# ChenyangQiQi/FateZero

Hardware: NVIDIA H100
Metric: edited frames/sec (512x512x8f, 50 DDIM steps: inversion + attention-fused edit) (higher is better)
Workload: dtype f16 (fp32 accumulate)

## Files before the change

### fatezero_b200/_build.py

```python
from __future__ import annotations

import os
import subprocess
import sys

HERE = os.path.dirname(os.path.abspath(__file__))
CSRC = os.path.join(HERE, "csrc")
LIB = os.path.join(HERE, "libfatezero_b200.so")
SOURCES = ["fz_capi.cu", "fz_gemm.cu", "fz_elem.cu", "fz_attn.cu", "fz_p2p.cu", "fz_clip.cu"]
ARCH = ["-gencode", "arch=compute_90a,code=sm_90a"]
NVCC_FLAGS = [*ARCH, "-lineinfo", "-O3", "-std=c++17", "-Xcompiler", "-fPIC",
              "--use_fast_math" if False else "-DFZ_NO_FAST_MATH"]


def _nvcc() -> str:
    for cand in (os.environ.get("NVCC"), "/usr/local/cuda/bin/nvcc", "nvcc"):
        if cand and (os.path.isabs(cand) and os.path.exists(cand) or not os.path.isabs(cand)):
            return cand
    return "nvcc"


def needs_build() -> bool:
    if not os.path.exists(LIB):
        return True
    t = os.path.getmtime(LIB)
    deps = [os.path.join(CSRC, f) for f in os.listdir(CSRC)] + [os.path.join(HERE, "..", "include", "fatezero_b200.h")]
    return any(os.path.getmtime(d) > t for d in deps if os.path.exists(d))


def build(force: bool = False, verbose: bool = True, variant: str = "", extra_flags=()) -> str:
    if variant:
        return _build(os.path.join(HERE, f"libfatezero_b200_{variant}.so"), os.path.join(HERE, "build", variant), list(extra_flags), verbose)
    if not force and not needs_build():
        return LIB
    return _build(LIB, os.path.join(HERE, "build"), [], verbose)


def _build(lib: str, objdir: str, extra_flags, verbose: bool) -> str:
    objs = []
    procs = []
    os.makedirs(objdir, exist_ok=True)
    for src in SOURCES:
        obj = os.path.join(objdir, src.replace(".cu", ".o"))
        cmd = [_nvcc(), *NVCC_FLAGS, *extra_flags, "-c", os.path.join(CSRC, src), "-o", obj]
        if verbose:
            print(" ".join(cmd), flush=True)
        procs.append((src, subprocess.Popen(cmd, stdout=subprocess.PIPE, stderr=subprocess.STDOUT)))
        objs.append(obj)
    for src, p in procs:
        out, _ = p.communicate()
        if p.returncode != 0:
            raise RuntimeError(f"nvcc failed on {src}:\n{out.decode()}")
    cmd = [_nvcc(), "-shared", "-o", lib, *objs, *ARCH]
    if verbose:
        print(" ".join(cmd), flush=True)
    subprocess.check_call(cmd)
    return lib


if __name__ == "__main__":
    import argparse
    ap = argparse.ArgumentParser()
    ap.add_argument("--force", action="store_true")
    ap.add_argument("--variant", default="")
    ap.add_argument("--flags", default="")
    a = ap.parse_args()
    print(build(force=a.force, variant=a.variant, extra_flags=a.flags.split()))
```

### fatezero_b200/csrc/fz_common.cuh

```cuda
#pragma once
#include <cuda.h>
#include <cuda_fp16.h>
#include <cuda_runtime.h>
#include <stdint.h>
#include <stdio.h>

namespace fz {

void set_error(const char* fmt, ...);
int check_single_device();
#define FZ_OK 0
#define FZ_ERR_INVALID 1
#define FZ_ERR_CUDA 2
#define FZ_CHECK_ARG(cond, ...)                        \
  do {                                                 \
    if (!(cond)) {                                     \
      ::fz::set_error(__VA_ARGS__);                    \
      return FZ_ERR_INVALID;                           \
    }                                                  \
  } while (0)
#define FZ_CUDA(expr)                                                                           \
  do {                                                                                          \
    cudaError_t _e = (expr);                                                                    \
    if (_e != cudaSuccess) {                                                                    \
      ::fz::set_error("%s failed: %s (%s:%d)", #expr, cudaGetErrorString(_e), __FILE__, __LINE__); \
      return FZ_ERR_CUDA;                                                                       \
    }                                                                                           \
  } while (0)

#ifdef __CUDACC__

__device__ __forceinline__ uint32_t smem_u32(const void* p) { return static_cast<uint32_t>(__cvta_generic_to_shared(p)); }

__device__ __forceinline__ void pdl_wait() { asm volatile("griddepcontrol.wait;" ::: "memory"); }
__device__ __forceinline__ void pdl_launch_dependents() { asm volatile("griddepcontrol.launch_dependents;" ::: "memory"); }

__device__ __forceinline__ bool elect_one() {
  uint32_t pred = 0;
  asm volatile(
      "{\n\t.reg .pred P1;\n\telect.sync _|P1, 0xffffffff;\n\tselp.u32 %0, 1, 0, P1;\n\t}\n"
      : "=r"(pred));
  return pred != 0;
}

__device__ __forceinline__ void mbar_init(uint64_t* bar, uint32_t count) {
  asm volatile("mbarrier.init.shared::cta.b64 [%0], %1;" ::"r"(smem_u32(bar)), "r"(count) : "memory");
}
__device__ __forceinline__ void fence_mbar_init() { asm volatile("fence.mbarrier_init.release.cluster;" ::: "memory"); }
__device__ __forceinline__ void mbar_expect_tx(uint64_t* bar, uint32_t bytes) {
  asm volatile("mbarrier.arrive.expect_tx.shared::cta.b64 _, [%0], %1;" ::"r"(smem_u32(bar)), "r"(bytes) : "memory");
}
__device__ __forceinline__ void mbar_arrive(uint64_t* bar) {
  asm volatile("mbarrier.arrive.shared::cta.b64 _, [%0];" ::"r"(smem_u32(bar)) : "memory");
}
__device__ __forceinline__ bool mbar_try_wait(uint64_t* bar, uint32_t parity) {
  uint32_t ok;
  asm volatile(
      "{\n\t.reg .pred p;\n\tmbarrier.try_wait.parity.shared::cta.b64 p, [%1], %2;\n\tselp.u32 %0, 1, 0, p;\n\t}\n"
      : "=r"(ok)
      : "r"(smem_u32(bar)), "r"(parity)
      : "memory");
  return ok != 0;
}
#ifndef FZ_MBAR_TIMEOUT_NS
#define FZ_MBAR_TIMEOUT_NS 2000000000ull
#endif
__device__ __forceinline__ uint64_t global_timer_ns() {
  uint64_t t;
  asm volatile("mov.u64 %0, %%globaltimer;" : "=l"(t));
  return t;
}
__device__ __forceinline__ void mbar_wait(uint64_t* bar, uint32_t parity) {
  if (mbar_try_wait(bar, parity)) return;
  const uint64_t t0 = global_timer_ns();
  while (!mbar_try_wait(bar, parity))
    if (global_timer_ns() - t0 > FZ_MBAR_TIMEOUT_NS) __trap();
}

__device__ __forceinline__ void fence_proxy_async_smem() { asm volatile("fence.proxy.async.shared::cta;" ::: "memory"); }

__device__ __forceinline__ void tma_prefetch_desc(const CUtensorMap* m) {
  asm volatile("prefetch.tensormap [%0];" ::"l"(reinterpret_cast<uint64_t>(m)) : "memory");
}
__device__ __forceinline__ void tma_load_2d(void* dst, const CUtensorMap* m, uint64_t* bar, int c0, int c1) {
  asm volatile(
      "cp.async.bulk.tensor.2d.shared::cluster.global.mbarrier::complete_tx::bytes [%0], [%1, {%3, %4}], [%2];" ::"r"(
          smem_u32(dst)),
      "l"(reinterpret_cast<uint64_t>(m)), "r"(smem_u32(bar)), "r"(c0), "r"(c1)
      : "memory");
}
__device__ __forceinline__ void tma_load_3d(void* dst, const CUtensorMap* m, uint64_t* bar, int c0, int c1, int c2) {
  asm volatile(
      "cp.async.bulk.tensor.3d.shared::cluster.global.mbarrier::complete_tx::bytes [%0], [%1, {%3, %4, %5}], [%2];" ::"r"(
          smem_u32(dst)),
      "l"(reinterpret_cast<uint64_t>(m)), "r"(smem_u32(bar)), "r"(c0), "r"(c1), "r"(c2)
      : "memory");
}
__device__ __forceinline__ void tma_load_4d(void* dst, const CUtensorMap* m, uint64_t* bar, int c0, int c1, int c2, int c3) {
  asm volatile(
      "cp.async.bulk.tensor.4d.shared::cluster.global.mbarrier::complete_tx::bytes [%0], [%1, {%3, %4, %5, %6}], [%2];" ::"r"(
          smem_u32(dst)),
      "l"(reinterpret_cast<uint64_t>(m)), "r"(smem_u32(bar)), "r"(c0), "r"(c1), "r"(c2), "r"(c3)
      : "memory");
}
__device__ __forceinline__ void tma_load_5d(void* dst, const CUtensorMap* m, uint64_t* bar, int c0, int c1, int c2, int c3,
                                            int c4) {
  asm volatile(
      "cp.async.bulk.tensor.5d.shared::cluster.global.mbarrier::complete_tx::bytes [%0], [%1, {%3, %4, %5, %6, %7}], "
      "[%2];" ::"r"(smem_u32(dst)),
      "l"(reinterpret_cast<uint64_t>(m)), "r"(smem_u32(bar)), "r"(c0), "r"(c1), "r"(c2), "r"(c3), "r"(c4)
      : "memory");
}
__device__ __forceinline__ void tma_store_2d(const CUtensorMap* m, const void* src, int c0, int c1) {
  asm volatile("cp.async.bulk.tensor.2d.global.shared::cta.bulk_group [%0, {%2, %3}], [%1];" ::"l"(reinterpret_cast<uint64_t>(m)),
               "r"(smem_u32(src)), "r"(c0), "r"(c1)
               : "memory");
}
__device__ __forceinline__ void tma_store_4d(const CUtensorMap* m, const void* src, int c0, int c1, int c2, int c3) {
  asm volatile("cp.async.bulk.tensor.4d.global.shared::cta.bulk_group [%0, {%2, %3, %4, %5}], [%1];" ::"l"(
                   reinterpret_cast<uint64_t>(m)),
               "r"(smem_u32(src)), "r"(c0), "r"(c1), "r"(c2), "r"(c3)
               : "memory");
}
__device__ __forceinline__ void tma_store_5d(const CUtensorMap* m, const void* src, int c0, int c1, int c2, int c3, int c4) {
  asm volatile("cp.async.bulk.tensor.5d.global.shared::cta.bulk_group [%0, {%2, %3, %4, %5, %6}], [%1];" ::"l"(
                   reinterpret_cast<uint64_t>(m)),
               "r"(smem_u32(src)), "r"(c0), "r"(c1), "r"(c2), "r"(c3), "r"(c4)
               : "memory");
}
__device__ __forceinline__ void tma_store_commit() { asm volatile("cp.async.bulk.commit_group;" ::: "memory"); }
template <int N>
__device__ __forceinline__ void tma_store_wait_read() {
  asm volatile("cp.async.bulk.wait_group.read %0;" ::"n"(N) : "memory");
}
template <int N>
__device__ __forceinline__ void tma_store_wait_all() {
  asm volatile("cp.async.bulk.wait_group %0;" ::"n"(N) : "memory");
}

__device__ __forceinline__ uint64_t wgmma_desc_k_sw128(uint32_t smem_addr) {
  uint64_t d = 0;
  d |= static_cast<uint64_t>((smem_addr & 0x3FFFF) >> 4);
  d |= static_cast<uint64_t>(1) << 16;
  d |= static_cast<uint64_t>(1024 >> 4) << 32;
  d |= static_cast<uint64_t>(1) << 62;
  return d;
}
__device__ __forceinline__ void named_bar_sync(int id, int n) { asm volatile("bar.sync %0, %1;" ::"r"(id), "r"(n) : "memory"); }

#endif

template <typename... KArgs, typename... Args>
inline cudaError_t launch_pdl(void (*kernel)(KArgs...), dim3 grid, dim3 block, size_t smem, cudaStream_t stream, Args&&... args) {
  cudaLaunchConfig_t cfg = {};
  cfg.gridDim = grid;
  cfg.blockDim = block;
  cfg.dynamicSmemBytes = smem;
  cfg.stream = stream;
  cudaLaunchAttribute attr[1];
  attr[0].id = cudaLaunchAttributeProgrammaticStreamSerialization;
  attr[0].val.programmaticStreamSerializationAllowed = 1;
  cfg.attrs = attr;
  cfg.numAttrs = 1;
  return cudaLaunchKernelEx(&cfg, kernel, static_cast<KArgs>(args)...);
}

int encode_tmap_f16(CUtensorMap* out, const void* base, int rank, const uint64_t* dims, const uint64_t* strides_elems,
                    const uint32_t* box, bool swizzle128);
int encode_tmap_f16_sw(CUtensorMap* out, const void* base, int rank, const uint64_t* dims, const uint64_t* strides_elems,
                       const uint32_t* box, int swizzle_bytes);

}
```

### fatezero_b200/csrc/fz_gemm.cu

```cuda
#include "fz_common.cuh"
#include "fz_wgmma.cuh"

#include <algorithm>
#include <climits>
#include <cstdio>
#include <cstring>

#include "../../include/fatezero_b200.h"

namespace fz {

constexpr int kMaxTaps = 9;
constexpr int kBlockM = 128;
constexpr int kBlockK = 64;
constexpr int kATileBytes = kBlockM * kBlockK * 2;

struct TapGemmParams {
  CUtensorMap tmA;
  CUtensorMap tmB;
  CUtensorMap tmR[2];
  CUtensorMap tmE;
  int n_res;
  int res_kblocks;
  int a_rank;
  int M, N;
  int rows_per_tile;
  int a_box_bytes;
  int k_blocks;
  int num_taps;
  int n_tiles, m_tiles;
  int ndecomp;
  int dimsz[4];
  int tap_off[kMaxTaps][5];
  const float* bias;
  const float* group_bias;
  int rows_per_group;
  const __half* residual;
  long long ldr;
  const __half* residual2;
  long long ldr2;
  __half* out;
  long long ldo;
  int mode;
  int vt_col_start;
  __half* out_vt;
  int vt_S, vt_d, vt_heads, vt_ld;
};

template <int BLOCK_N>
struct TapGemmCfg {
  static constexpr int kBTileBytes = BLOCK_N * kBlockK * 2;
  static constexpr int kBTilePad = (kBTileBytes + 1023) / 1024 * 1024;
  static constexpr int kStageBytes = kATileBytes + kBTilePad;
  static constexpr int kStagesRaw = (227 * 1024 - 1280) / kStageBytes;
  static constexpr int kStages = kStagesRaw > 8 ? 8 : kStagesRaw;
  static constexpr int kSmemBytes = kStages * kStageBytes + 1024  + 256 ;
};

__device__ __forceinline__ float gelu_erf(float x) {
  const float z = fabsf(x) * 0.70710678118654752f;
  float t, e;
  asm("rcp.approx.ftz.f32 %0, %1;" : "=f"(t) : "f"(fmaf(0.3275911f, z, 1.0f)));
  float poly = fmaf(1.061405429f, t, -1.453152027f);
  poly = fmaf(poly, t, 1.421413741f);
  poly = fmaf(poly, t, -0.284496736f);
  poly = fmaf(poly, t, 0.254829592f);
  asm("ex2.approx.ftz.f32 %0, %1;" : "=f"(e) : "f"(-1.4426950408889634f * z * z));
  const float erf_abs = fmaf(-poly * t, e, 1.0f);
  return 0.5f * x * (1.0f + copysignf(erf_abs, x));
}

__device__ __forceinline__ void epi_store1(const TapGemmParams& p, long long m, int col, float v, const float* gb) {
  if (p.bias) v += __ldg(p.bias + col);
  if (col >= p.vt_col_start) {
    const long long bf = m / p.vt_S;
    const int s = static_cast<int>(m % p.vt_S);
    const int cv = col - p.vt_col_start;
    p.out_vt[((bf * p.vt_heads + cv / p.vt_d) * p.vt_d + cv % p.vt_d) * p.vt_ld + s] = __float2half_rn(v);
  } else {
    if (gb) v += __ldg(gb + col);
    if (p.residual) v += __half2float(p.residual[m * p.ldr + col]);
    if (p.residual2) v += __half2float(p.residual2[m * p.ldr2 + col]);
    p.out[m * p.ldo + col] = __float2half_rn(v);
  }
}

template <int BLOCK_N>
__global__ void __launch_bounds__(384, 1) tapgemm_kernel(const __grid_constant__ TapGemmParams p) {
  using Cfg = TapGemmCfg<BLOCK_N>;
  extern __shared__ uint8_t smem_raw[];
  uint8_t* smem = reinterpret_cast<uint8_t*>((reinterpret_cast<uintptr_t>(smem_raw) + 1023) & ~uintptr_t(1023));
  uint64_t* bars = reinterpret_cast<uint64_t*>(smem + Cfg::kStages * Cfg::kStageBytes);
  uint64_t* full = bars;
  uint64_t* empty = bars + Cfg::kStages;

  const int wg = threadIdx.x >> 7;
  pdl_launch_dependents();
  const int num_tiles = p.m_tiles * p.n_tiles;
  const int k_iters = p.num_taps * p.k_blocks + p.n_res * p.res_kblocks;

  if (threadIdx.x == 0) {
    tma_prefetch_desc(&p.tmA);
    tma_prefetch_desc(&p.tmB);
    for (int s = 0; s < Cfg::kStages; ++s) {
      mbar_init(&full[s], 1);
      mbar_init(&empty[s], 8);
    }
    fence_mbar_init();
  }
  __syncthreads();
  pdl_wait();

  if (wg == 2) {
    if (threadIdx.x == 256) {
      int stage = 0;
      uint32_t phase = 0;
      for (int tile = blockIdx.x; tile < num_tiles; tile += gridDim.x) {
        const int mt = tile / p.n_tiles, nt = tile % p.n_tiles;
        int rem = mt * p.rows_per_tile;
        int base[5] = {0, 0, 0, 0, 0};
        for (int d = 0; d < p.ndecomp; ++d) {
          base[d + 1] = rem % p.dimsz[d];
          rem /= p.dimsz[d];
        }
        const int n0 = nt * BLOCK_N;
        for (int tap = 0; tap < p.num_taps; ++tap) {
          const int c1 = base[1] + p.tap_off[tap][1], c2 = base[2] + p.tap_off[tap][2];
          const int c3 = base[3] + p.tap_off[tap][3], c4 = base[4] + p.tap_off[tap][4];
          for (int kb = 0; kb < p.k_blocks; ++kb) {
            mbar_wait(&empty[stage], phase ^ 1);
            uint8_t* sa = smem + stage * Cfg::kStageBytes;
            uint8_t* sb = sa + kATileBytes;
            mbar_expect_tx(&full[stage], p.a_box_bytes + Cfg::kBTileBytes);
            const int c0 = kb * kBlockK + p.tap_off[tap][0];
            switch (p.a_rank) {
              case 2: tma_load_2d(sa, &p.tmA, &full[stage], c0, c1); break;
              case 3: tma_load_3d(sa, &p.tmA, &full[stage], c0, c1, c2); break;
              case 4: tma_load_4d(sa, &p.tmA, &full[stage], c0, c1, c2, c3); break;
              default: tma_load_5d(sa, &p.tmA, &full[stage], c0, c1, c2, c3, c4); break;
            }
            tma_load_3d(sb, &p.tmB, &full[stage], kb * kBlockK, n0, tap);
            if (++stage == Cfg::kStages) { stage = 0; phase ^= 1; }
          }
        }
        for (int r = 0; r < p.n_res; ++r) {
          for (int j = 0; j < p.res_kblocks; ++j) {
            mbar_wait(&empty[stage], phase ^ 1);
            uint8_t* sa = smem + stage * Cfg::kStageBytes;
            uint8_t* sb = sa + kATileBytes;
            mbar_expect_tx(&full[stage], kATileBytes + Cfg::kBTileBytes);
            tma_load_2d(sa, &p.tmR[r], &full[stage], n0 + j * kBlockK, mt * p.rows_per_tile);
            tma_load_3d(sb, &p.tmE, &full[stage], 0, 0, j);
            if (++stage == Cfg::kStages) { stage = 0; phase ^= 1; }
          }
        }
      }
    }
    return;
  }

  const int lane = threadIdx.x & 31;
  const int warp_in = (threadIdx.x >> 5) & 3;
  const uint64_t desc0 = wgmma_desc_k_sw128(smem_u32(smem));
  float acc[BLOCK_N / 2];
  int stage = 0;
  uint32_t phase = 0;
  const int r_base = wg * 64 + warp_in * 16 + (lane >> 2);
  const int c_base = 2 * (lane & 3);
  const bool pair_ok = (p.ldo % 2) == 0 && (reinterpret_cast<uintptr_t>(p.out) & 3) == 0;
  for (int tile = blockIdx.x; tile < num_tiles; tile += gridDim.x) {
    const int mt = tile / p.n_tiles, nt = tile % p.n_tiles;
    int prev = -1;
    for (int it = 0; it < k_iters; ++it) {
      mbar_wait(&full[stage], phase);
      const uint64_t da = desc0 + static_cast<uint32_t>((stage * Cfg::kStageBytes + wg * 64 * 128) >> 4);
      const uint64_t db = desc0 + static_cast<uint32_t>((stage * Cfg::kStageBytes + kATileBytes) >> 4);
      wgmma_fence();
#pragma unroll
      for (int k = 0; k < kBlockK / 16; ++k) wgmma_f16<BLOCK_N>(acc, da + 2 * k, db + 2 * k, (it | k) ? 1u : 0u);
      wgmma_commit();
      wgmma_wait<1>();
      if (prev >= 0 && lane == 0) mbar_arrive(&empty[prev]);
      prev = stage;
      if (++stage == Cfg::kStages) { stage = 0; phase ^= 1; }
    }
    wgmma_wait<0>();
    if (prev >= 0 && lane == 0) mbar_arrive(&empty[prev]);

#pragma unroll
    for (int h = 0; h < 2; ++h) {
      const int r = r_base + 8 * h;
      const long long m = static_cast<long long>(mt) * p.rows_per_tile + r;
      if (r >= p.rows_per_tile || m >= p.M) continue;
      if (p.mode == FZ_EPI_GEGLU) {
        constexpr int HALF = BLOCK_N / 2;
        if constexpr (HALF % 8 == 0) {
          __half* orow = p.out + m * p.ldo;
#pragma unroll
          for (int i = 0; i < HALF / 8; ++i) {
            const int c = 8 * i + c_base;
            const int oc = nt * HALF + c;
            if (oc >= p.N) continue;
            float x0 = acc[4 * i + 2 * h], x1 = acc[4 * i + 2 * h + 1];
            float g0 = acc[4 * (i + HALF / 8) + 2 * h], g1 = acc[4 * (i + HALF / 8) + 2 * h + 1];
            if (p.bias) {
              const float* b = p.bias + nt * BLOCK_N + c;
              x0 += __ldg(b); x1 += __ldg(b + 1); g0 += __ldg(b + HALF); g1 += __ldg(b + HALF + 1);
            }
            const float o0 = x0 * gelu_erf(g0), o1 = x1 * gelu_erf(g1);
            if (pair_ok && oc + 1 < p.N) {
              *reinterpret_cast<__half2*>(orow + oc) = __floats2half2_rn(o0, o1);
            } else {
              orow[oc] = __float2half_rn(o0);
              if (oc + 1 < p.N) orow[oc + 1] = __float2half_rn(o1);
            }
          }
        }
      } else {
        const float* gb = p.group_bias ? p.group_bias + (m / p.rows_per_group) * p.N : nullptr;
        __half* orow = p.out + m * p.ldo;
#pragma unroll
        for (int i = 0; i < BLOCK_N / 8; ++i) {
          const int col = nt * BLOCK_N + 8 * i + c_base;
          if (col >= p.N) continue;
          float v0 = acc[4 * i + 2 * h], v1 = acc[4 * i + 2 * h + 1];
          if (pair_ok && col + 2 <= p.N && col + 2 <= p.vt_col_start) {
            if (p.bias) { v0 += __ldg(p.bias + col); v1 += __ldg(p.bias + col + 1); }
            if (gb) { v0 += __ldg(gb + col); v1 += __ldg(gb + col + 1); }
            if (p.residual) { v0 += __half2float(p.residual[m * p.ldr + col]); v1 += __half2float(p.residual[m * p.ldr + col + 1]); }
            if (p.residual2) { v0 += __half2float(p.residual2[m * p.ldr2 + col]); v1 += __half2float(p.residual2[m * p.ldr2 + col + 1]); }
            *reinterpret_cast<__half2*>(orow + col) = __floats2half2_rn(v0, v1);
          } else {
            epi_store1(p, m, col, v0, gb);
            if (col + 1 < p.N) epi_store1(p, m, col + 1, v1, gb);
          }
        }
      }
    }
  }
}

static int g_num_sms = 0;
static int num_sms() {
  if (g_num_sms == 0) {
    int dev = 0;
    cudaGetDevice(&dev);
    cudaDeviceGetAttribute(&g_num_sms, cudaDevAttrMultiProcessorCount, dev);
    if (g_num_sms <= 0) g_num_sms = 132;
  }
  return g_num_sms;
}

template <int BN>
static int launch_tapgemm(const TapGemmParams& p, cudaStream_t stream) {
  using Cfg = TapGemmCfg<BN>;
  static bool configured = false;
  if (!configured) {
    FZ_CUDA(cudaFuncSetAttribute(tapgemm_kernel<BN>, cudaFuncAttributeMaxDynamicSharedMemorySize, Cfg::kSmemBytes));
    configured = true;
  }
  const int tiles = p.m_tiles * p.n_tiles;
  const int grid = std::min(tiles, num_sms());
  FZ_CUDA(launch_pdl(tapgemm_kernel<BN>, dim3(grid), dim3(384), Cfg::kSmemBytes, stream, p));
  FZ_CUDA(cudaGetLastError());
  return FZ_OK;
}

static int n_foldable(const TapGemmParams& p) {
  if (p.mode != FZ_EPI_ROWMAJOR || p.vt_col_start != INT_MAX) return 0;
  const __half* rs[2] = {p.residual, p.residual2};
  const long long lds[2] = {p.ldr, p.ldr2};
  int n = 0;
  for (int i = 0; i < 2; ++i) {
    if (!rs[i]) continue;
    if ((reinterpret_cast<uintptr_t>(rs[i]) & 15) != 0 || lds[i] % 8 != 0) return 0;
    ++n;
  }
  return n;
}

static int pick_block_n(const TapGemmParams& p, int gemm_cols, int forced, int m_tiles, int k_main) {
  if (forced > 0) return forced;
  static const int cands[] = {256, 160, 128, 64, 32, 16};
  if (p.mode == FZ_EPI_GEGLU) return (gemm_cols % 256 == 0) ? 256 : ((gemm_cols % 160 == 0) ? 160 : ((gemm_cols % 128 == 0) ? 128 : ((gemm_cols % 64 == 0) ? 64 : 32)));
  const int sms = num_sms();
  const int n_fold = n_foldable(p);
  int best = 16;
  double best_cost = 1e30;
  for (int bn : cands) {
    const long long n_tiles = (gemm_cols + bn - 1) / bn;
    const long long tiles = n_tiles * m_tiles;
    const long long waves = (tiles + sms - 1) / sms;
    const double k = k_main + n_fold * ((bn + kBlockK - 1) / kBlockK);
    const double cost = static_cast<double>(waves) * (bn * k + 24.0 * bn + 110.0 * k + 0.15 * bn * bn);
    if (cost < best_cost - 1e-9) { best_cost = cost; best = bn; }
  }
  return best;
}

__device__ __half g_eye[4][256][64];
__global__ void eye_init_kernel() {
  for (int i = blockIdx.x * blockDim.x + threadIdx.x; i < 4 * 256 * 64; i += gridDim.x * blockDim.x) {
    const int k = i % 64, n = (i / 64) % 256, j = i / (64 * 256);
    (&g_eye[0][0][0])[i] = __float2half_rn(n == 64 * j + k ? 1.f : 0.f);
  }
}

static int eye_table(__half** out, cudaStream_t stream) {
  static __half* eye = nullptr;
  if (!eye) {
    cudaStreamCaptureStatus cs = cudaStreamCaptureStatusNone;
    FZ_CUDA(cudaStreamIsCapturing(stream, &cs));
    FZ_CHECK_ARG(cs == cudaStreamCaptureStatusNone, "fz_init() must run once before the library is used under CUDA-graph capture");
    __half* e = nullptr;
    FZ_CUDA(cudaGetSymbolAddress(reinterpret_cast<void**>(&e), g_eye));
    eye_init_kernel<<<64, 256, 0, stream>>>();
    FZ_CUDA(cudaGetLastError());
    FZ_CUDA(cudaStreamSynchronize(stream));
    eye = e;
  }
  *out = eye;
  return FZ_OK;
}

static int fold_residuals(TapGemmParams& p, int bn, cudaStream_t stream) {
  p.n_res = 0;
  p.res_kblocks = 0;
  if (n_foldable(p) == 0) return FZ_OK;
  const __half* rs[2] = {p.residual, p.residual2};
  const long long lds[2] = {p.ldr, p.ldr2};
  __half* eye = nullptr;
  if (int rc = eye_table(&eye, stream)) return rc;
  {
    uint64_t dims[3] = {64, 256, 4};
    uint64_t strides[2] = {64, 64 * 256};
    uint32_t box[3] = {64, static_cast<uint32_t>(bn), 1};
    if (int rc = encode_tmap_f16(&p.tmE, eye, 3, dims, strides, box, true)) return rc;
  }
  for (int i = 0; i < 2; ++i) {
    if (!rs[i]) continue;
    uint64_t dims[2] = {static_cast<uint64_t>(p.N), static_cast<uint64_t>(p.M)};
    uint64_t strides[1] = {static_cast<uint64_t>(lds[i])};
    uint32_t box[2] = {kBlockK, kBlockM};
    if (int rc = encode_tmap_f16(&p.tmR[p.n_res], rs[i], 2, dims, strides, box, true)) return rc;
    ++p.n_res;
  }
  p.res_kblocks = (bn + kBlockK - 1) / kBlockK;
  p.residual = nullptr;
  p.residual2 = nullptr;
  return FZ_OK;
}

static int dispatch_tapgemm(TapGemmParams& p, int gemm_cols, int bn, cudaStream_t stream) {
  if (int rc = check_single_device()) return rc;
  p.n_tiles = (gemm_cols + bn - 1) / bn;
  if (int rc = fold_residuals(p, bn, stream)) return rc;
  switch (bn) {
    case 256: return launch_tapgemm<256>(p, stream);
    case 160: return launch_tapgemm<160>(p, stream);
    case 128: return launch_tapgemm<128>(p, stream);
    case 64: return launch_tapgemm<64>(p, stream);
    case 32: return launch_tapgemm<32>(p, stream);
    case 16: return launch_tapgemm<16>(p, stream);
    default: set_error("unsupported BLOCK_N %d", bn); return FZ_ERR_INVALID;
  }
}

static int fill_epilogue(TapGemmParams& p, const fz_epilogue_t* e, int M, int gemm_cols) {
  p.bias = nullptr; p.group_bias = nullptr; p.rows_per_group = 1; p.residual = nullptr; p.ldr = 0; p.residual2 = nullptr; p.ldr2 = 0;
  p.mode = FZ_EPI_ROWMAJOR; p.vt_col_start = INT_MAX; p.out_vt = nullptr; p.vt_S = p.vt_d = p.vt_heads = p.vt_ld = 1;
  p.N = gemm_cols;
  if (!e) return FZ_OK;
  p.bias = e->bias; p.group_bias = e->group_bias; p.rows_per_group = e->rows_per_group > 0 ? e->rows_per_group : 1;
  p.residual = static_cast<const __half*>(e->residual); p.ldr = e->ldr;
  p.residual2 = static_cast<const __half*>(e->residual2); p.ldr2 = e->ldr2;
  p.mode = e->mode;
  if (e->mode == FZ_EPI_GEGLU) {
    FZ_CHECK_ARG(gemm_cols % 2 == 0, "GEGLU needs an even number of GEMM columns");
    FZ_CHECK_ARG(!e->residual && !e->residual2 && !e->group_bias && !e->out_vt,
                 "GEGLU epilogue takes no residual, group bias or V^T output");
    p.N = gemm_cols / 2;
  }
  if (e->out_vt) {
    FZ_CHECK_ARG(e->vt_S > 0 && e->vt_d > 0 && e->vt_heads > 0 && M % e->vt_S == 0, "bad V^T geometry");
    p.vt_col_start = e->vt_col_start; p.out_vt = static_cast<__half*>(e->out_vt);
    p.vt_S = e->vt_S; p.vt_d = e->vt_d; p.vt_heads = e->vt_heads; p.vt_ld = e->vt_ld > 0 ? e->vt_ld : e->vt_S;
  }
  return FZ_OK;
}

}

using namespace fz;

extern "C" int fz_init(cudaStream_t stream) {
  if (int rc = check_single_device()) return rc;
  __half* eye = nullptr;
  return eye_table(&eye, stream);
}

extern "C" int fz_gemm_f16(const void* A, long long lda, const void* W, long long ldw, int M, int N, int K, const fz_epilogue_t* epi,
                           void* out, long long ldo, int force_block_n, cudaStream_t stream) {
  FZ_CHECK_ARG(A && W && out, "fz_gemm_f16: null pointer");
  FZ_CHECK_ARG(M > 0 && N > 0 && K > 0, "fz_gemm_f16: bad shape %d %d %d", M, N, K);
  FZ_CHECK_ARG(lda % 8 == 0 && ldw % 8 == 0 && K % 8 == 0, "fz_gemm_f16: lda/ldw/K must be multiples of 8 (16-byte TMA strides)");
  TapGemmParams p;
  memset(&p, 0, sizeof(p));
  {
    uint64_t dims[2] = {static_cast<uint64_t>(K), static_cast<uint64_t>(M)};
    uint64_t strides[1] = {static_cast<uint64_t>(lda)};
    uint32_t box[2] = {kBlockK, kBlockM};
    if (int rc = encode_tmap_f16(&p.tmA, A, 2, dims, strides, box, true)) return rc;
  }
  const int rc0 = fill_epilogue(p, epi, M, N);
  if (rc0) return rc0;
  p.m_tiles = (M + kBlockM - 1) / kBlockM;
  const int bn = pick_block_n(p, N, force_block_n, p.m_tiles, (K + kBlockK - 1) / kBlockK);
  {
    uint64_t dims[3] = {static_cast<uint64_t>(K), static_cast<uint64_t>(N), 1};
    uint64_t strides[2] = {static_cast<uint64_t>(ldw), static_cast<uint64_t>(ldw) * N};
    uint32_t box[3] = {kBlockK, static_cast<uint32_t>(bn), 1};
    if (int rc = encode_tmap_f16(&p.tmB, W, 3, dims, strides, box, true)) return rc;
  }
  p.a_rank = 2; p.M = M; p.rows_per_tile = kBlockM; p.a_box_bytes = kATileBytes;
  p.k_blocks = (K + kBlockK - 1) / kBlockK; p.num_taps = 1;
  p.m_tiles = (M + kBlockM - 1) / kBlockM;
  p.ndecomp = 1; p.dimsz[0] = INT_MAX;
  p.out = static_cast<__half*>(out); p.ldo = ldo;
  return dispatch_tapgemm(p, N, bn, stream);
}

static int conv3x3_impl(const void* x, long long ldx, int NB, int H, int W, int Cin, const void* w, int Cout, int stride, int asym_pad,
                        const fz_epilogue_t* epi, void* out, long long ldo, int force_block_n, cudaStream_t stream) {
  FZ_CHECK_ARG(x && w && out, "fz_conv3x3: null pointer");
  FZ_CHECK_ARG(stride == 1 || stride == 2, "fz_conv3x3: stride must be 1 or 2");
  FZ_CHECK_ARG(Cin % 8 == 0 && ldx % 8 == 0, "fz_conv3x3: Cin/ldx must be multiples of 8");
  FZ_CHECK_ARG(stride == 1 || (H % 2 == 0 && W % 2 == 0), "fz_conv3x3: stride 2 needs even H, W");
  const int Ho = H / stride, Wo = W / stride;
  FZ_CHECK_ARG(!asym_pad || stride == 2, "fz_conv3x3: asymmetric padding is the stride-2 downsample variant");
  int bw = std::min(Wo, 128);
  while (Wo % bw) --bw;
  FZ_CHECK_ARG(Wo <= 128 || bw >= 8, "fz_conv3x3: output width %d has no divisor in [8, 128] to tile its rows with", Wo);
  int bh = (bw == Wo) ? std::min(Ho, 128 / bw) : 1;
  while (Ho % bh) --bh;
  int bn_img = (bh == Ho) ? std::min(NB, 128 / (bw * bh)) : 1;
  while (NB % bn_img) --bn_img;
  TapGemmParams p;
  memset(&p, 0, sizeof(p));
  const int M = NB * Ho * Wo;
  const int rc0 = fill_epilogue(p, epi, M, Cout);
  if (rc0) return rc0;
  if (stride == 1) {
    uint64_t dims[4] = {(uint64_t)Cin, (uint64_t)W, (uint64_t)H, (uint64_t)NB};
    uint64_t strides[3] = {(uint64_t)ldx, (uint64_t)ldx * W, (uint64_t)ldx * W * H};
    uint32_t box[4] = {kBlockK, (uint32_t)bw, (uint32_t)bh, (uint32_t)bn_img};
    if (int rc = encode_tmap_f16(&p.tmA, x, 4, dims, strides, box, true)) return rc;
    p.a_rank = 4;
    for (int t = 0; t < 9; ++t) {
      p.tap_off[t][0] = 0; p.tap_off[t][1] = t % 3 - 1; p.tap_off[t][2] = t / 3 - 1; p.tap_off[t][3] = 0; p.tap_off[t][4] = 0;
    }
  } else {
    uint64_t dims[5] = {(uint64_t)(ldx + Cin), (uint64_t)Wo, (uint64_t)Ho, (uint64_t)NB, 2};
    uint64_t strides[4] = {(uint64_t)2 * ldx, (uint64_t)2 * ldx * W, (uint64_t)ldx * W * H, (uint64_t)ldx * W};
    uint32_t box[5] = {kBlockK, (uint32_t)bw, (uint32_t)bh, (uint32_t)bn_img, 1};
    if (int rc = encode_tmap_f16(&p.tmA, x, 5, dims, strides, box, true)) return rc;
    p.a_rank = 5;
    for (int t = 0; t < 9; ++t) {
      const int ky = t / 3, kx = t % 3;
      const int py = asym_pad ? (ky & 1) : ((ky == 1) ? 0 : 1), px = asym_pad ? (kx & 1) : ((kx == 1) ? 0 : 1);
      p.tap_off[t][0] = px * (int)ldx;
      p.tap_off[t][1] = asym_pad ? (kx >> 1) : ((kx == 0) ? -1 : 0);
      p.tap_off[t][2] = asym_pad ? (ky >> 1) : ((ky == 0) ? -1 : 0);
      p.tap_off[t][3] = 0;
      p.tap_off[t][4] = py;
    }
  }
  p.rows_per_tile = bw * bh * bn_img;
  p.m_tiles = M / p.rows_per_tile;
  const int bn = pick_block_n(p, Cout, force_block_n, p.m_tiles, 9 * ((Cin + kBlockK - 1) / kBlockK));
  {
    uint64_t dims[3] = {(uint64_t)Cin, (uint64_t)Cout, 9};
    uint64_t strides[2] = {(uint64_t)Cin, (uint64_t)Cin * Cout};
    uint32_t box[3] = {kBlockK, (uint32_t)bn, 1};
    if (int rc = encode_tmap_f16(&p.tmB, w, 3, dims, strides, box, true)) return rc;
  }
  p.M = M; p.rows_per_tile = bw * bh * bn_img; p.a_box_bytes = p.rows_per_tile * 128;
  p.k_blocks = (Cin + kBlockK - 1) / kBlockK; p.num_taps = 9;
  p.m_tiles = M / p.rows_per_tile;
  p.ndecomp = 3; p.dimsz[0] = Wo; p.dimsz[1] = Ho; p.dimsz[2] = NB;
  p.out = static_cast<__half*>(out); p.ldo = ldo;
  return dispatch_tapgemm(p, Cout, bn, stream);
}

extern "C" int fz_conv3x3_nhwc_f16(const void* x, long long ldx, int NB, int H, int W, int Cin, const void* w, int Cout, int stride,
                                   const fz_epilogue_t* epi, void* out, long long ldo, int force_block_n, cudaStream_t stream) {
  return conv3x3_impl(x, ldx, NB, H, W, Cin, w, Cout, stride, 0, epi, out, ldo, force_block_n, stream);
}

extern "C" int fz_conv3x3_down_asym_nhwc_f16(const void* x, long long ldx, int NB, int H, int W, int Cin, const void* w, int Cout,
                                             const fz_epilogue_t* epi, void* out, long long ldo, int force_block_n, cudaStream_t stream) {
  return conv3x3_impl(x, ldx, NB, H, W, Cin, w, Cout, 2, 1, epi, out, ldo, force_block_n, stream);
}

static int tconv3_impl(const void* x, long long ldx, int B, int F, int HW, int Cin, const void* w, int Cout, const fz_epilogue_t* epi,
                       void* out, long long ldo, int force_block_n, int halo, cudaStream_t stream) {
  FZ_CHECK_ARG(x && w && out, "fz_tconv3: null pointer");
  FZ_CHECK_ARG(Cin % 8 == 0 && ldx % 8 == 0, "fz_tconv3: Cin/ldx must be multiples of 8");
  int bp = std::min(HW, 128);
  while (HW % bp) --bp;
  int bf = (bp == HW) ? std::min(F, 128 / bp) : 1;
  while (F % bf) --bf;
  TapGemmParams p;
  memset(&p, 0, sizeof(p));
  const int M = B * F * HW;
  const int rc0 = fill_epilogue(p, epi, M, Cout);
  if (rc0) return rc0;
  const int Fx = F + 2 * halo;
  {
    uint64_t dims[4] = {(uint64_t)Cin, (uint64_t)HW, (uint64_t)Fx, (uint64_t)B};
    uint64_t strides[3] = {(uint64_t)ldx, (uint64_t)ldx * HW, (uint64_t)ldx * HW * Fx};
    uint32_t box[4] = {kBlockK, (uint32_t)bp, (uint32_t)bf, 1};
    if (int rc = encode_tmap_f16(&p.tmA, x, 4, dims, strides, box, true)) return rc;
  }
  p.a_rank = 4;
  for (int t = 0; t < 3; ++t) { p.tap_off[t][2] = t - 1 + halo; }
  p.rows_per_tile = bp * bf;
  p.m_tiles = M / p.rows_per_tile;
  const int bn = pick_block_n(p, Cout, force_block_n, p.m_tiles, 3 * ((Cin + kBlockK - 1) / kBlockK));
  {
    uint64_t dims[3] = {(uint64_t)Cin, (uint64_t)Cout, 3};
    uint64_t strides[2] = {(uint64_t)Cin, (uint64_t)Cin * Cout};
    uint32_t box[3] = {kBlockK, (uint32_t)bn, 1};
    if (int rc = encode_tmap_f16(&p.tmB, w, 3, dims, strides, box, true)) return rc;
  }
  p.M = M; p.rows_per_tile = bp * bf; p.a_box_bytes = p.rows_per_tile * 128;
  p.k_blocks = (Cin + kBlockK - 1) / kBlockK; p.num_taps = 3;
  p.m_tiles = M / p.rows_per_tile;
  p.ndecomp = 3; p.dimsz[0] = HW; p.dimsz[1] = F; p.dimsz[2] = B;
  p.out = static_cast<__half*>(out); p.ldo = ldo;
  return dispatch_tapgemm(p, Cout, bn, stream);
}

extern "C" int fz_tconv3_f16(const void* x, long long ldx, int B, int F, int HW, int Cin, const void* w, int Cout, const fz_epilogue_t* epi,
                             void* out, long long ldo, int force_block_n, cudaStream_t stream) {
  return tconv3_impl(x, ldx, B, F, HW, Cin, w, Cout, epi, out, ldo, force_block_n, 0, stream);
}

extern "C" int fz_tconv3_halo_f16(const void* x_ext, long long ldx, int B, int F, int HW, int Cin, const void* w, int Cout,
                                  const fz_epilogue_t* epi, void* out, long long ldo, int force_block_n, cudaStream_t stream) {
  return tconv3_impl(x_ext, ldx, B, F, HW, Cin, w, Cout, epi, out, ldo, force_block_n, 1, stream);
}
```

Before: 1.458.

## Add ping-pong consumer warpgroups and register reallocation to TMA GEMM

Restructures the persistent wgmma GEMM so that, for BLOCK_N up to 160, each consumer warpgroup handles the full 128-row tile on alternating tiles. Named barriers order the two warpgroups so one's epilogue overlaps the other's MMA main loop. It also adds setmaxnreg to give producer registers to the consumers, precomputes the transposed-V row offset in the epilogue, and retunes the block-N cost model while dropping 256 for non-GEGLU modes. The risks are doubled accumulator register pressure, a more complex barrier and phase protocol, and different tile choices.

```diff
diff --git a/fatezero_b200/_build.py b/fatezero_b200/_build.py
--- a/fatezero_b200/_build.py
+++ b/fatezero_b200/_build.py
@@ -28,21 +28,23 @@
     return any(os.path.getmtime(d) > t for d in deps if os.path.exists(d))
 
 
-def build(force: bool = False, verbose: bool = True, variant: str = "", extra_flags=()) -> str:
+def build(force: bool = False, verbose: bool = True, variant: str = "", extra_flags=(), src_dir: str = "") -> str:
     if variant:
-        return _build(os.path.join(HERE, f"libfatezero_b200_{variant}.so"), os.path.join(HERE, "build", variant), list(extra_flags), verbose)
+        return _build(os.path.join(HERE, f"libfatezero_b200_{variant}.so"), os.path.join(HERE, "build", variant), list(extra_flags), verbose,
+                      src_dir)
     if not force and not needs_build():
         return LIB
     return _build(LIB, os.path.join(HERE, "build"), [], verbose)
 
 
-def _build(lib: str, objdir: str, extra_flags, verbose: bool) -> str:
+def _build(lib: str, objdir: str, extra_flags, verbose: bool, src_dir: str = "") -> str:
     objs = []
     procs = []
     os.makedirs(objdir, exist_ok=True)
     for src in SOURCES:
         obj = os.path.join(objdir, src.replace(".cu", ".o"))
-        cmd = [_nvcc(), *NVCC_FLAGS, *extra_flags, "-c", os.path.join(CSRC, src), "-o", obj]
+        path = os.path.join(src_dir, src) if src_dir and os.path.exists(os.path.join(src_dir, src)) else os.path.join(CSRC, src)
+        cmd = [_nvcc(), *NVCC_FLAGS, *extra_flags, "-I", CSRC, "-c", path, "-o", obj]
         if verbose:
             print(" ".join(cmd), flush=True)
         procs.append((src, subprocess.Popen(cmd, stdout=subprocess.PIPE, stderr=subprocess.STDOUT)))
@@ -64,5 +66,6 @@
     ap.add_argument("--force", action="store_true")
     ap.add_argument("--variant", default="")
     ap.add_argument("--flags", default="")
+    ap.add_argument("--src-dir", default="")
     a = ap.parse_args()
-    print(build(force=a.force, variant=a.variant, extra_flags=a.flags.split()))
+    print(build(force=a.force, variant=a.variant, extra_flags=a.flags.split(), src_dir=a.src_dir))
diff --git a/fatezero_b200/csrc/fz_common.cuh b/fatezero_b200/csrc/fz_common.cuh
--- a/fatezero_b200/csrc/fz_common.cuh
+++ b/fatezero_b200/csrc/fz_common.cuh
@@ -147,6 +147,12 @@
   return d;
 }
 __device__ __forceinline__ void named_bar_sync(int id, int n) { asm volatile("bar.sync %0, %1;" ::"r"(id), "r"(n) : "memory"); }
+__device__ __forceinline__ void named_bar_arrive(int id, int n) { asm volatile("bar.arrive %0, %1;" ::"r"(id), "r"(n) : "memory"); }
+
+template <int N>
+__device__ __forceinline__ void setmaxnreg_dec() { asm volatile("setmaxnreg.dec.sync.aligned.u32 %0;" ::"n"(N)); }
+template <int N>
+__device__ __forceinline__ void setmaxnreg_inc() { asm volatile("setmaxnreg.inc.sync.aligned.u32 %0;" ::"n"(N)); }
 
 #endif
 
diff --git a/fatezero_b200/csrc/fz_gemm.cu b/fatezero_b200/csrc/fz_gemm.cu
--- a/fatezero_b200/csrc/fz_gemm.cu
+++ b/fatezero_b200/csrc/fz_gemm.cu
@@ -70,13 +70,10 @@
   return 0.5f * x * (1.0f + copysignf(erf_abs, x));
 }
 
-__device__ __forceinline__ void epi_store1(const TapGemmParams& p, long long m, int col, float v, const float* gb) {
+__device__ __forceinline__ void epi_store1(const TapGemmParams& p, long long m, int col, float v, const float* gb, long long vt_row) {
   if (p.bias) v += __ldg(p.bias + col);
   if (col >= p.vt_col_start) {
-    const long long bf = m / p.vt_S;
-    const int s = static_cast<int>(m % p.vt_S);
-    const int cv = col - p.vt_col_start;
-    p.out_vt[((bf * p.vt_heads + cv / p.vt_d) * p.vt_d + cv % p.vt_d) * p.vt_ld + s] = __float2half_rn(v);
+    p.out_vt[vt_row + static_cast<long long>(col - p.vt_col_start) * p.vt_ld] = __float2half_rn(v);
   } else {
     if (gb) v += __ldg(gb + col);
     if (p.residual) v += __half2float(p.residual[m * p.ldr + col]);
@@ -86,8 +83,67 @@
 }
 
 template <int BLOCK_N>
+__device__ __forceinline__ void tile_epilogue(const TapGemmParams& p, const float* acc, int mt, int nt, int r_base, int c_base,
+                                              bool pair_ok) {
+#pragma unroll
+  for (int h = 0; h < 2; ++h) {
+    const int r = r_base + 8 * h;
+    const long long m = static_cast<long long>(mt) * p.rows_per_tile + r;
+    if (r >= p.rows_per_tile || m >= p.M) continue;
+    if (p.mode == FZ_EPI_GEGLU) {
+      constexpr int HALF = BLOCK_N / 2;
+      if constexpr (HALF % 8 == 0) {
+        __half* orow = p.out + m * p.ldo;
+#pragma unroll
+        for (int i = 0; i < HALF / 8; ++i) {
+          const int c = 8 * i + c_base;
+          const int oc = nt * HALF + c;
+          if (oc >= p.N) continue;
+          float x0 = acc[4 * i + 2 * h], x1 = acc[4 * i + 2 * h + 1];
+          float g0 = acc[4 * (i + HALF / 8) + 2 * h], g1 = acc[4 * (i + HALF / 8) + 2 * h + 1];
+          if (p.bias) {
+            const float* b = p.bias + nt * BLOCK_N + c;
+            x0 += __ldg(b); x1 += __ldg(b + 1); g0 += __ldg(b + HALF); g1 += __ldg(b + HALF + 1);
+          }
+          const float o0 = x0 * gelu_erf(g0), o1 = x1 * gelu_erf(g1);
+          if (pair_ok && oc + 1 < p.N) {
+            *reinterpret_cast<__half2*>(orow + oc) = __floats2half2_rn(o0, o1);
+          } else {
+            orow[oc] = __float2half_rn(o0);
+            if (oc + 1 < p.N) orow[oc + 1] = __float2half_rn(o1);
+          }
+        }
+      }
+    } else {
+      const float* gb = p.group_bias ? p.group_bias + (m / p.rows_per_group) * p.N : nullptr;
+      const long long vt_row = p.out_vt ? (m / p.vt_S) * p.vt_heads * p.vt_d * p.vt_ld + m % p.vt_S : 0;
+      __half* orow = p.out + m * p.ldo;
+#pragma unroll
+      for (int i = 0; i < BLOCK_N / 8; ++i) {
+        const int col = nt * BLOCK_N + 8 * i + c_base;
+        if (col >= p.N) continue;
+        float v0 = acc[4 * i + 2 * h], v1 = acc[4 * i + 2 * h + 1];
+        if (pair_ok && col + 2 <= p.N && col + 2 <= p.vt_col_start) {
+          if (p.bias) { v0 += __ldg(p.bias + col); v1 += __ldg(p.bias + col + 1); }
+          if (gb) { v0 += __ldg(gb + col); v1 += __ldg(gb + col + 1); }
+          if (p.residual) { v0 += __half2float(p.residual[m * p.ldr + col]); v1 += __half2float(p.residual[m * p.ldr + col + 1]); }
+          if (p.residual2) { v0 += __half2float(p.residual2[m * p.ldr2 + col]); v1 += __half2float(p.residual2[m * p.ldr2 + col + 1]); }
+          *reinterpret_cast<__half2*>(orow + col) = __floats2half2_rn(v0, v1);
+        } else {
+          epi_store1(p, m, col, v0, gb, vt_row);
+          if (col + 1 < p.N) epi_store1(p, m, col + 1, v1, gb, vt_row);
+        }
+      }
+    }
+  }
+}
+
+template <int BLOCK_N>
 __global__ void __launch_bounds__(384, 1) tapgemm_kernel(const __grid_constant__ TapGemmParams p) {
   using Cfg = TapGemmCfg<BLOCK_N>;
+  constexpr bool kPingPong = BLOCK_N <= 160;
+  constexpr int kRowBlocks = kPingPong ? 2 : 1;
+  constexpr bool kRegSplit = BLOCK_N >= 128;
   extern __shared__ uint8_t smem_raw[];
   uint8_t* smem = reinterpret_cast<uint8_t*>((reinterpret_cast<uintptr_t>(smem_raw) + 1023) & ~uintptr_t(1023));
   uint64_t* bars = reinterpret_cast<uint64_t*>(smem + Cfg::kStages * Cfg::kStageBytes);
@@ -104,7 +160,7 @@
     tma_prefetch_desc(&p.tmB);
     for (int s = 0; s < Cfg::kStages; ++s) {
       mbar_init(&full[s], 1);
-      mbar_init(&empty[s], 8);
+      mbar_init(&empty[s], kPingPong ? 4 : 8);
     }
     fence_mbar_init();
   }
@@ -112,6 +168,7 @@
   pdl_wait();
 
   if (wg == 2) {
+    if constexpr (kRegSplit) setmaxnreg_dec<40>();
     if (threadIdx.x == 256) {
       int stage = 0;
       uint32_t phase = 0;
@@ -159,84 +216,59 @@
     return;
   }
 
+  if constexpr (kRegSplit) setmaxnreg_inc<232>();
   const int lane = threadIdx.x & 31;
   const int warp_in = (threadIdx.x >> 5) & 3;
   const uint64_t desc0 = wgmma_desc_k_sw128(smem_u32(smem));
-  float acc[BLOCK_N / 2];
+  float acc[kRowBlocks * BLOCK_N / 2];
+  const int row0 = kPingPong ? 0 : wg * 64;
+  const int c_base = 2 * (lane & 3);
+  const bool pair_ok = (p.ldo % 2) == 0 && (reinterpret_cast<uintptr_t>(p.out) & 3) == 0;
   int stage = 0;
   uint32_t phase = 0;
-  const int r_base = wg * 64 + warp_in * 16 + (lane >> 2);
-  const int c_base = 2 * (lane & 3);
-  const bool pair_ok = (p.ldo % 2) == 0 && (reinterpret_cast<uintptr_t>(p.out) & 3) == 0;
-  for (int tile = blockIdx.x; tile < num_tiles; tile += gridDim.x) {
+  auto skip_other_tile = [&]() {
+    const int s = stage + k_iters;
+    phase ^= (s / Cfg::kStages) & 1;
+    stage = s % Cfg::kStages;
+  };
+  if (kPingPong && wg == 1) skip_other_tile();
+  const int first = blockIdx.x + (kPingPong ? wg * gridDim.x : 0);
+  const int stride = kPingPong ? 2 * gridDim.x : gridDim.x;
+  for (int tile = first; tile < num_tiles; tile += stride) {
     const int mt = tile / p.n_tiles, nt = tile % p.n_tiles;
+    if (kPingPong && tile >= blockIdx.x + gridDim.x) {
+      if (wg == 0) named_bar_sync(1, 256);
+      else named_bar_sync(2, 256);
+    }
     int prev = -1;
     for (int it = 0; it < k_iters; ++it) {
       mbar_wait(&full[stage], phase);
-      const uint64_t da = desc0 + static_cast<uint32_t>((stage * Cfg::kStageBytes + wg * 64 * 128) >> 4);
+      const uint64_t da = desc0 + static_cast<uint32_t>((stage * Cfg::kStageBytes + row0 * 128) >> 4);
       const uint64_t db = desc0 + static_cast<uint32_t>((stage * Cfg::kStageBytes + kATileBytes) >> 4);
       wgmma_fence();
 #pragma unroll
-      for (int k = 0; k < kBlockK / 16; ++k) wgmma_f16<BLOCK_N>(acc, da + 2 * k, db + 2 * k, (it | k) ? 1u : 0u);
+      for (int k = 0; k < kBlockK / 16; ++k) {
+#pragma unroll
+        for (int b = 0; b < kRowBlocks; ++b)
+          wgmma_f16<BLOCK_N>(acc + b * (BLOCK_N / 2), da + b * (64 * 128 / 16) + 2 * k, db + 2 * k, (it | k) ? 1u : 0u);
+      }
       wgmma_commit();
       wgmma_wait<1>();
       if (prev >= 0 && lane == 0) mbar_arrive(&empty[prev]);
       prev = stage;
       if (++stage == Cfg::kStages) { stage = 0; phase ^= 1; }
     }
+    if (kPingPong && tile + gridDim.x < num_tiles) {
+      if (wg == 0) named_bar_arrive(2, 256);
+      else named_bar_arrive(1, 256);
+    }
     wgmma_wait<0>();
     if (prev >= 0 && lane == 0) mbar_arrive(&empty[prev]);
 
 #pragma unroll
-    for (int h = 0; h < 2; ++h) {
-      const int r = r_base + 8 * h;
-      const long long m = static_cast<long long>(mt) * p.rows_per_tile + r;
-      if (r >= p.rows_per_tile || m >= p.M) continue;
-      if (p.mode == FZ_EPI_GEGLU) {
-        constexpr int HALF = BLOCK_N / 2;
-        if constexpr (HALF % 8 == 0) {
-          __half* orow = p.out + m * p.ldo;
-#pragma unroll
-          for (int i = 0; i < HALF / 8; ++i) {
-            const int c = 8 * i + c_base;
-            const int oc = nt * HALF + c;
-            if (oc >= p.N) continue;
-            float x0 = acc[4 * i + 2 * h], x1 = acc[4 * i + 2 * h + 1];
-            float g0 = acc[4 * (i + HALF / 8) + 2 * h], g1 = acc[4 * (i + HALF / 8) + 2 * h + 1];
-            if (p.bias) {
-              const float* b = p.bias + nt * BLOCK_N + c;
-              x0 += __ldg(b); x1 += __ldg(b + 1); g0 += __ldg(b + HALF); g1 += __ldg(b + HALF + 1);
-            }
-            const float o0 = x0 * gelu_erf(g0), o1 = x1 * gelu_erf(g1);
-            if (pair_ok && oc + 1 < p.N) {
-              *reinterpret_cast<__half2*>(orow + oc) = __floats2half2_rn(o0, o1);
-            } else {
-              orow[oc] = __float2half_rn(o0);
-              if (oc + 1 < p.N) orow[oc + 1] = __float2half_rn(o1);
-            }
-          }
-        }
-      } else {
-        const float* gb = p.group_bias ? p.group_bias + (m / p.rows_per_group) * p.N : nullptr;
-        __half* orow = p.out + m * p.ldo;
-#pragma unroll
-        for (int i = 0; i < BLOCK_N / 8; ++i) {
-          const int col = nt * BLOCK_N + 8 * i + c_base;
-          if (col >= p.N) continue;
-          float v0 = acc[4 * i + 2 * h], v1 = acc[4 * i + 2 * h + 1];
-          if (pair_ok && col + 2 <= p.N && col + 2 <= p.vt_col_start) {
-            if (p.bias) { v0 += __ldg(p.bias + col); v1 += __ldg(p.bias + col + 1); }
-            if (gb) { v0 += __ldg(gb + col); v1 += __ldg(gb + col + 1); }
-            if (p.residual) { v0 += __half2float(p.residual[m * p.ldr + col]); v1 += __half2float(p.residual[m * p.ldr + col + 1]); }
-            if (p.residual2) { v0 += __half2float(p.residual2[m * p.ldr2 + col]); v1 += __half2float(p.residual2[m * p.ldr2 + col + 1]); }
-            *reinterpret_cast<__half2*>(orow + col) = __floats2half2_rn(v0, v1);
-          } else {
-            epi_store1(p, m, col, v0, gb);
-            if (col + 1 < p.N) epi_store1(p, m, col + 1, v1, gb);
-          }
-        }
-      }
-    }
+    for (int b = 0; b < kRowBlocks; ++b)
+      tile_epilogue<BLOCK_N>(p, acc + b * (BLOCK_N / 2), mt, nt, row0 + 64 * b + warp_in * 16 + (lane >> 2), c_base, pair_ok);
+    if (kPingPong) skip_other_tile();
   }
 }
 
@@ -281,8 +313,8 @@
 
 static int pick_block_n(const TapGemmParams& p, int gemm_cols, int forced, int m_tiles, int k_main) {
   if (forced > 0) return forced;
-  static const int cands[] = {256, 160, 128, 64, 32, 16};
   if (p.mode == FZ_EPI_GEGLU) return (gemm_cols % 256 == 0) ? 256 : ((gemm_cols % 160 == 0) ? 160 : ((gemm_cols % 128 == 0) ? 128 : ((gemm_cols % 64 == 0) ? 64 : 32)));
+  static const int cands[] = {160, 128, 64, 32, 16};
   const int sms = num_sms();
   const int n_fold = n_foldable(p);
   int best = 16;
@@ -292,7 +324,7 @@
     const long long tiles = n_tiles * m_tiles;
     const long long waves = (tiles + sms - 1) / sms;
     const double k = k_main + n_fold * ((bn + kBlockK - 1) / kBlockK);
-    const double cost = static_cast<double>(waves) * (bn * k + 24.0 * bn + 110.0 * k + 0.15 * bn * bn);
+    const double cost = static_cast<double>(waves + 1) * (bn * k + 1270.0 * k + 2.7 * bn * bn + 5500.0);
     if (cost < best_cost - 1e-9) { best_cost = cost; best = bn; }
   }
   return best;
```

New measurement: 1.478 (median of 6 runs). 1.01x the previous value.
